# sacs-epfl/decentralizepy

Measured on AMD Instinct MI355X. Metric: GiB/s fp32 params encoded+decoded (device-resident), 1% top-k, higher is better.
Workload: dtype f32

## Files before the change

decentralizepy_amd/csrc/dpz_topk.h:

```cpp
#pragma once
#include <cstdlib>

#include "dpz_common.h"
#include "dpz_replace.h"

namespace dpz {

struct KeySrc {
  const float* x;
  const float* x0;
  float* acc;
  int mode;
  int rekey;
};

struct Raw4 {
  float4 a, b, q;
  int cnt;
};

template <bool VEC, bool ACC = true>
__device__ __forceinline__ void load_raw4(const KeySrc& s, int64_t i0, int64_t n, Raw4& r) {
  const int64_t rem = n - i0;
  r.cnt = rem >= 4 ? 4 : (rem > 0 ? (int)rem : 0);
// ... 89 lines not shown
constexpr int EX_HIST_BLOCKS = 1024;
constexpr int SMP_N = 65536;
constexpr int SMP_CHUNK = 64;
constexpr int SMP_NCHUNK = SMP_N / SMP_CHUNK;
constexpr int CB_SHIFT = 20;
constexpr int CB = 2048;
#ifndef DPZ_HB
#define DPZ_HB 1024
#endif
constexpr int HB = DPZ_HB;
constexpr int HBR = HB + 1;
static_assert(HB % 256 == 0 && HB <= 1024, "fine bins: multiple of 256, at most 1024");
#ifndef DPZ_WMAX
#define DPZ_WMAX 8192
#endif
#ifndef DPZ_WMIN_RANGE
#define DPZ_WMIN_RANGE 1024
#endif
#ifndef DPZ_FG
#define DPZ_FG 2
#endif
constexpr int W_MAX = DPZ_WMAX;
#ifndef DPZ_WSMALL
#define DPZ_WSMALL 3072
#endif
constexpr int W_SMALL = DPZ_WSMALL;
constexpr int64_t W_SMALL_N = (1 << 24) + (1 << 22);
#ifndef DPZ_WPIPE
#define DPZ_WPIPE 4096
#endif
constexpr int W_PIPE = DPZ_WPIPE;
constexpr int64_t W_PIPE_N = 1 << 24;
enum : int { GEOM_LONE = 0, GEOM_SHARED = 1, GEOM_PIPE = 2 };
constexpr int FG = DPZ_FG;
#ifndef DPZ_FOCC
#define DPZ_FOCC 8
#endif
constexpr int FOCC = DPZ_FOCC;
constexpr int W_MIN_RANGE = DPZ_WMIN_RANGE;
#ifndef DPZ_GH_COPIES
#define DPZ_GH_COPIES 8
#endif
constexpr int GH_COPIES = DPZ_GH_COPIES;
constexpr int GH_STRIDE = HB + 16;
constexpr int SEL_SEGS = 32;
constexpr int SEL_LCAP = 1024;
constexpr int NSUB = 16;
constexpr int SUBCAP = 256;
constexpr int BCAP = NSUB * SUBCAP;
constexpr int RANK_MAX = 1024;
constexpr int B_MAX = W_MAX / 4;
constexpr int STAGE = 256;
constexpr uint32_t DENSE = 0xFFFFFFFFu;

struct FastGeom {
  int64_t W;
  int64_t B;
  int64_t R;
  int64_t CAP;
};

static inline FastGeom fast_geom(int64_t n, int64_t k = 0, int geom = GEOM_LONE) {
  FastGeom g;
  int64_t W = (n + W_MIN_RANGE - 1) / W_MIN_RANGE;
  const int64_t wlone = DPZ_KNOB_INT(WLONE, 0);
  const int64_t wpipe_knob = DPZ_KNOB_INT(WPIPE, 0);
  const int64_t wpipe = (wpipe_knob > 0 && wpipe_knob <= W_MAX)
                            ? wpipe_knob
                            : (n >= W_PIPE_N ? (int64_t)W_PIPE : (int64_t)W_SMALL);
  const int64_t wmax = (geom != GEOM_LONE && n <= W_SMALL_N)
                           ? (geom == GEOM_PIPE ? wpipe : (int64_t)W_SMALL)
                           : ((wlone > 0 && wlone < W_MAX) ? wlone : W_MAX);
  if (W > wmax) W = wmax;
  if (W < 1) W = 1;
  int64_t R = (n + W - 1) / W;
  R = (R + 31) & ~int64_t(31);
  W = (n + R - 1) / R;
  int64_t cap = ((R / 4) + 63) & ~int64_t(63);
  if (k > n / 16) {
    const double frac = 1.25 * (double)k / (double)n + 0.05;
    cap = ((int64_t)(frac * (double)R) + 63) & ~int64_t(63);
    if (cap > ((R + 63) & ~int64_t(63))) cap = (R + 63) & ~int64_t(63);
  }
  if (cap < 64) cap = 64;
  if (k <= n / 16 && cap > 1024) cap = 1024;
  g.W = W; g.B = (W + 3) / 4; g.R = R; g.CAP = cap;
  return g;
}

static inline size_t align256(size_t v) { return (v + 255) & ~size_t(255); }

struct WsLayout {
  size_t ctrl, chist, ex_hist, ex_gt, ex_eq, ex_off, ex_eqb;
  size_t f_ghist, f_segcnt, f_blkabove, f_blkoff, f_cidx, f_ckey, f_cval, f_blcnt, f_blkey, f_blidx;
  size_t total;
  int64_t ex_nblk;
  FastGeom fg;
};

static inline WsLayout ws_layout(int64_t n, int64_t k = 0, int geom = GEOM_LONE) {
  WsLayout L;
  size_t o = 0;
  L.ex_nblk = (n + EX_CHUNK - 1) / EX_CHUNK;
  if (L.ex_nblk < 1) L.ex_nblk = 1;
  L.fg = fast_geom(n > 0 ? n : 1, k, geom);
  L.ctrl = o; o += align256(sizeof(TopkCtrl));
  L.chist = o; o += align256(CB * 4);
  L.ex_hist = o; o += align256(4096 * 4);
  L.ex_gt = o; o += align256(L.ex_nblk * 4);
  L.ex_eq = o; o += align256(L.ex_nblk * 4);
  L.ex_off = o; o += align256(L.ex_nblk * 4);
  L.ex_eqb = o; o += align256(L.ex_nblk * 4);
  L.f_ghist = o; o += align256(GH_COPIES * GH_STRIDE * 4);
  L.f_blcnt = o; o += align256(NSUB * 4);
  L.f_segcnt = o; o += align256(L.fg.W * 4);
  L.f_blkabove = o; o += align256(L.fg.B * 4);
  L.f_blkoff = o; o += align256(L.fg.B * 4);
  L.f_cidx = o; o += align256((size_t)L.fg.W * L.fg.CAP * 4);
  L.f_ckey = o; o += align256((size_t)L.fg.W * L.fg.CAP * 4);
  L.f_cval = o; o += align256((size_t)L.fg.W * L.fg.CAP * 4);
  L.f_blkey = o; o += align256((size_t)BCAP * 4);
  L.f_blidx = o; o += align256((size_t)BCAP * 4);
  L.total = o;
  return L;
}

static inline size_t ws_bytes_needed(int64_t n, int64_t k) {
  size_t m = 0;
  for (int geom = GEOM_LONE; geom <= GEOM_PIPE; ++geom) {
    const size_t t = ws_layout(n, k, geom).total;
    if (t > m) m = t;
  }
  return m;
}

struct EncodeArgs {
  const float* x; const float* x0; float* acc; int acc_mode; const float* vals_src;
  int64_t n, k; int32_t* idx_out; float* val_out; int32_t* counter; char* ws;
  hipStream_t st;
  const ReplaceJob* job;
  int32_t* status_out;
  bool shared;
  int val_h;
  const FoldBase* fbase;
  float* base_out;
  uint32_t* selmask;
  uint32_t* planes;
  uint32_t hint_sig;
  bool keep_x;
};
static inline uint32_t hint_signature(int64_t n, int64_t k, int geom, int acc_mode, bool x0) {
  uint64_t h = 1469598103934665603ull;
  const uint64_t v[5] = {(uint64_t)n, (uint64_t)k, (uint64_t)geom, (uint64_t)acc_mode,
                         x0 ? 1ull : 0ull};
  for (int i = 0; i < 5; ++i) h = (h ^ v[i]) * 1099511628211ull;
  return (uint32_t)(h ^ (h >> 32)) | 1u;
}
#ifndef DPZ_HINT_DELTA
#define DPZ_HINT_DELTA 0.0625f
#endif
constexpr float HINT_LO = 1.0f - DPZ_HINT_DELTA, HINT_HI = 1.0f + DPZ_HINT_DELTA;
constexpr int64_t SL_RMAX = 8192;
static inline int64_t mask_words(int64_t n) { return (n + 31) >> 5; }
int sliced_from_idx(const EncodeArgs& a, const uint32_t* guard = nullptr);
bool fused_foldbase_ok(const EncodeArgs& a, bool vec);
int launch_fold_base(const float* x, int64_t n, const FoldBase& fb, float* out, hipStream_t st);

int run_exact(const EncodeArgs& a, const WsLayout& L, int rekey, bool vec, int keep_ties = 0,
              int64_t cap = 0);
int run_sampled(const EncodeArgs& a, const WsLayout& L, bool vec, int phases = 3);
int topk_encode_status(const float* x, const float* x0, float* acc, int acc_mode,
                       const float* vals_src, int64_t n, int64_t k, int32_t* idx_out,
                       float* val_out, int32_t* counter, void* ws, size_t ws_bytes,
// ... 25 lines not shown
```

decentralizepy_amd/csrc/dpz_topk_sampled.hip:

```cpp
#include <cstdio>
#include <cstdlib>

#include "dpz_topk.h"

namespace dpz {

#ifndef DPZ_FILTER_NT
#define DPZ_FILTER_NT 1
#endif

#ifdef DPZ_STAMPS
__device__ unsigned long long g_stamps[64];
#define STAMP_MIN(i) do { if (threadIdx.x == 0) atomicMin(&g_stamps[i], __builtin_amdgcn_s_memrealtime()); } while (0)
#define STAMP_MAX(i) do { __syncthreads(); if (threadIdx.x == 0) atomicMax(&g_stamps[i], __builtin_amdgcn_s_memrealtime()); } while (0)
#define STAMP_ONE(i) do { if (threadIdx.x == 0) g_stamps[i] = __builtin_amdgcn_s_memrealtime(); } while (0)
__device__ unsigned long long g_bst[16][4096];
#define STAMP_T0(i) do { if (threadIdx.x == 0 && blockIdx.x < 4096) g_bst[i][blockIdx.x] = __builtin_amdgcn_s_memrealtime(); } while (0)
__device__ unsigned long long g_fst[6][8192];
#define STAMP_W(i) do { const int64_t _sg = (int64_t)blockIdx.x * 4 + (threadIdx.x >> 6); if ((threadIdx.x & 63) == 0 && _sg < 8192) g_fst[i][_sg] = __builtin_amdgcn_s_memrealtime(); } while (0)
#else
#define STAMP_T0(i) do {} while (0)
#define STAMP_W(i) do {} while (0)
#define STAMP_MIN(i) do {} while (0)
#define STAMP_MAX(i) do {} while (0)
// ... 72 lines not shown
#pragma unroll
  for (int e = 0; e < 8; ++e) local += hv8[e];
  uint32_t tot;
  uint32_t before = block_excl_scan(local, wsum, &tot);
#pragma unroll
  for (int e = 0; e < 8; ++e) {
    const uint32_t bin = (uint32_t)(2047 - 8 * t - e);
    const uint32_t hv = hv8[e];
    if (r_lo <= (uint32_t)SMP_N && before < r_lo && r_lo <= before + hv) win[3] = bin;
    if (r_hi >= 1 && before < r_hi && r_hi <= before + hv) win[2] = bin;
    before += hv;
  }
  __syncthreads();
  if (t == 0) {
    const uint32_t blo = win[3], bhi = win[2];
    const uint32_t lo = (blo != 0xFFFFFFFFu) ? (blo << CB_SHIFT) : 0u;
    const uint64_t h64 = (bhi != 0xFFFFFFFFu) ? ((uint64_t)(bhi + 1) << CB_SHIFT) : (1ull << 31);
    const uint32_t hi = (uint32_t)(h64 > (1ull << 31) ? (1ull << 31) : h64);
    const uint32_t width = hi - lo;
    uint32_t sft = 0;
    while ((((uint64_t)width + (1ull << sft) - 1) >> sft) > (uint64_t)HB) ++sft;
    win[0] = lo;
    win[1] = hi;
    win[2] = sft;
  }
  __syncthreads();
}

static inline void window_ranks(int64_t n, int64_t k, uint32_t* r_lo, uint32_t* r_hi) {
  const double r_est = (double)k * SMP_N / (double)n;
  const double sd = sqrt(r_est);
  const double rlo_d = ceil(r_est + 6.0 * sd + 16.0);
  const double rhi_d = floor(r_est - 6.0 * sd - 16.0);
  *r_lo = rlo_d > SMP_N ? (uint32_t)SMP_N + 1 : (uint32_t)rlo_d;
  *r_hi = rhi_d < 1.0 ? 1u : (uint32_t)rhi_d;
}

struct WaveList {
  uint32_t* gidx;
  uint32_t* gkey;
  float* gval;
  uint32_t* stg;
  uint32_t staged;
  uint32_t flushed;

  __device__ __forceinline__ void flush(int lane, bool write, uint32_t* h, uint32_t lo, uint32_t hi,
                                        uint32_t shift) {
    __builtin_amdgcn_s_waitcnt(0xC07F);
    __builtin_amdgcn_wave_barrier();
    for (uint32_t j = lane; j < staged; j += 64) {
      const uint32_t key = stg[STAGE + j];
      atomicAdd(&h[fine_bin(key, lo, hi, shift)], 1u);
      if (write) {
        gidx[flushed + j] = stg[j];
        gkey[flushed + j] = key;
        if (gval) gval[flushed + j] = __uint_as_float(stg[2 * STAGE + j]);
      }
    }
    __builtin_amdgcn_wave_barrier();
    flushed += staged;
    staged = 0;
  }
};

template <bool VEC, bool ACC, int G>
__device__ __forceinline__ void load_groups(const KeySrc& s, int64_t base, int64_t end, int lane,
                                            Raw4 (&raw)[G]) {
  if (VEC && base + G * 256 <= end) {
    const bool rekey = ACC && s.mode == DPZ_ACC_ACCUMULATE && s.rekey;
#pragma unroll
    for (int q = 0; q < G; ++q) {
      const int64_t i0 = base + q * 256 + lane * 4;
      raw[q].cnt = 4;
      if (!rekey) {
#if DPZ_FILTER_NT
        typedef float v4f __attribute__((ext_vector_type(4)));
        const v4f va = __builtin_nontemporal_load(reinterpret_cast<const v4f*>(s.x + i0));
        raw[q].a = make_float4(va.x, va.y, va.z, va.w);
        if (s.x0) {
          const v4f vb = __builtin_nontemporal_load(reinterpret_cast<const v4f*>(s.x0 + i0));
          raw[q].b = make_float4(vb.x, vb.y, vb.z, vb.w);
        }
#else
        raw[q].a = *reinterpret_cast<const float4*>(s.x + i0);
        if (s.x0) raw[q].b = *reinterpret_cast<const float4*>(s.x0 + i0);
#endif
      }
      if (ACC && s.mode != DPZ_ACC_NONE) raw[q].q = *reinterpret_cast<const float4*>(s.acc + i0);
    }
  } else {
#pragma unroll
    for (int q = 0; q < G; ++q) {
      const int64_t i0 = base + q * 256 + lane * 4;
      raw[q].cnt = 0;
      if (i0 < end) load_raw4<VEC, ACC>(s, i0, end, raw[q]);
    }
  }
}

template <bool VEC, bool ACC, int G>
__global__ void __launch_bounds__(256, ACC ? 4 : FOCC) sampled_filter_kernel(
    KeySrc s, int64_t n, uint32_t r_lo, uint32_t r_hi, int64_t W, int64_t R, int64_t CAP,
    TopkCtrl* ctrl, const uint32_t* __restrict__ chist, uint32_t* ghist, uint32_t* segcnt,
    uint32_t* cidx, uint32_t* ckey, float* cval, float* __restrict__ copy_out) {
  __shared__ uint32_t h[HBR];
  __shared__ uint32_t win[4];
  __shared__ uint32_t wsum[16];
  __shared__ uint32_t st[4][3 * STAGE];
  STAMP_W(0);
  const int wid = threadIdx.x >> 6, lane = threadIdx.x & 63;
  for (int b = threadIdx.x; b < HBR; b += 256) h[b] = 0;
  const int64_t seg = (int64_t)blockIdx.x * 4 + wid;
  const int64_t beg = seg * R;
  const int64_t end = (beg + R < n) ? beg + R : n;
  const bool store_acc = (s.mode == DPZ_ACC_ACCUMULATE) && !s.rekey;
  uint4 cv[2];
  {
    const uint4* c4 = reinterpret_cast<const uint4*>(chist) + (510 - 2 * threadIdx.x);
    cv[0] = c4[0];
    cv[1] = c4[1];
  }
  Raw4 raw[G];
  load_groups<VEC, ACC, G>(s, beg, end, lane, raw);
  block_window(cv, r_lo, r_hi, win, wsum);
  STAMP_W(1);
  STAMP_W(2);
  const uint32_t lo = win[0], hi = win[1], shift = win[2];
  if (seg == 0 && lane == 0) {
    ctrl->lo = lo;
    ctrl->hi = hi;
    ctrl->shift = shift;
  }
  WaveList L{cidx + seg * CAP, ckey + seg * CAP, cval ? cval + seg * CAP : nullptr, st[wid], 0u,
             0u};
  uint32_t run = 0;
  bool dense = false;
  for (int64_t base = beg; base < end; base += G * 256) {
    if (base != beg) load_groups<VEC, ACC, G>(s, base, end, lane, raw);
#pragma unroll
    for (int q = 0; q < G; ++q) {
      uint32_t kq[4];
      const int cq = raw[q].cnt;
      if (copy_out) {
        const int64_t i0 = base + q * 256 + lane * 4;
        if (VEC && cq == 4) {
          typedef float v4f __attribute__((ext_vector_type(4)));
          const v4f v = {raw[q].a.x, raw[q].a.y, raw[q].a.z, raw[q].a.w};
          __builtin_nontemporal_store(v, reinterpret_cast<v4f*>(copy_out + i0));
        } else {
          const float xv[4] = {raw[q].a.x, raw[q].a.y, raw[q].a.z, raw[q].a.w};
#pragma unroll
          for (int e = 0; e < 4; ++e)
            if (e < cq) copy_out[i0 + e] = xv[e];
        }
      }
      if (cq) finish_keys4<VEC, ACC>(s, base + q * 256 + lane * 4, store_acc, raw[q], kq);
      bool f[4];
      uint32_t pre = 0, tot = 0;
#pragma unroll
      for (int e = 0; e < 4; ++e) {
        f[e] = e < cq && kq[e] >= lo;
        const uint64_t m = __ballot(f[e]);
        pre += mbcnt64(m);
        tot += (uint32_t)__popcll(m);
      }
      if (tot) {
        if (!dense && run + tot <= (uint32_t)CAP && tot <= (uint32_t)STAGE) {
          const uint32_t i0 = (uint32_t)(base + q * 256 + lane * 4);
          if (L.staged + tot > STAGE) L.flush(lane, true, h, lo, hi, shift);
          uint32_t p = L.staged + pre;
          const float xv[4] = {raw[q].a.x, raw[q].a.y, raw[q].a.z, raw[q].a.w};
#pragma unroll
          for (int e = 0; e < 4; ++e) {
            if (f[e]) {
              L.stg[p] = i0 + e;
              L.stg[STAGE + p] = kq[e];
              L.stg[2 * STAGE + p] = __float_as_uint(xv[e]);
              ++p;
            }
          }
          L.staged += tot;
        } else {
          if (!dense) L.flush(lane, false, h, lo, hi, shift);
          dense = true;
#pragma unroll
          for (int e = 0; e < 4; ++e)
            if (f[e]) atomicAdd(&h[fine_bin(kq[e], lo, hi, shift)], 1u);
// ... 108 lines not shown
  }
#pragma unroll
  for (int u = 0; u < D - 1; ++u) ld(u, u);
  if (hsig) {
    const bool ok = hS == hsig && hT > 0u && hT < 0x7F800000u;
    if (!ok) {
      if (BID == 0 && threadIdx.x == 0) {
        ctrl->status = 1;
        ctrl->hinted = 1;
        ctrl->val_h = (uint32_t)val_h;
      }
      if (CP != 0) {
        const int64_t ngc = (end4 - beg + 255) >> 8;
        for (int64_t j = 0; j < ngc; ++j) {
          const int64_t i0 = beg + j * 256 + lane * 4;
          if (i0 < end4) {
            const v4f a = xa[i0 >> 2];
            const v4f b = CP == 1 ? a : v4f{fb.of(a.x), fb.of(a.y), fb.of(a.z), fb.of(a.w)};
            __builtin_nontemporal_store(b, reinterpret_cast<v4f*>(copy_out) + (i0 >> 2));
          }
        }
        if (end4 < end && end4 + lane < end) {
          const float xv = s.x[end4 + lane];
          copy_out[end4 + lane] = CP == 1 ? xv : fb.of(xv);
        }
      }
      return;
    }
    if (BID == 0) {
      if (threadIdx.x < NSUB) blcnt[threadIdx.x] = 0;
      if (threadIdx.x == 0) {
        ctrl->status = 0;
        ctrl->nbound = 0;
        ctrl->val_h = (uint32_t)val_h;
        ctrl->hinted = 1;
      }
    }
  }
  uint32_t lo, hi, shift;
  if (hsig) {
    hint_window(hT, &lo, &hi, &shift);
  } else {
    block_window(cv, r_lo, r_hi, win, wsum);
    lo = win[0];
    hi = win[1];
    shift = win[2];
  }
  STAMP_T0(6);
  if (seg == 0 && lane == 0) {
    ctrl->lo = lo;
    ctrl->hi = hi;
    ctrl->shift = shift;
  }
  WaveList L{cidx + seg * CAP, ckey + seg * CAP, cval ? cval + seg * CAP : nullptr, M.st[wid], 0u,
             0u};
  uint32_t run = 0;
  bool dense = false;
  auto proc = [&](int64_t j, int u) {
    const int64_t i0 = beg + j * 256 + lane * 4;
    const int cq = i0 < end4 ? 4 : 0;
    if (CP == 1 && cq) __builtin_nontemporal_store(A[u], reinterpret_cast<v4f*>(copy_out) + (i0 >> 2));
    if (CP == 2 && cq) {
      const v4f b = {fb.of(A[u].x), fb.of(A[u].y), fb.of(A[u].z), fb.of(A[u].w)};
      __builtin_nontemporal_store(b, reinterpret_cast<v4f*>(copy_out) + (i0 >> 2));
    }
    const float xv[4] = {A[u].x, A[u].y, A[u].z, A[u].w};
    uint32_t kq[4];
    if (SRC == 1) {
      const float bv[4] = {B[u].x, B[u].y, B[u].z, B[u].w};
#pragma unroll
      for (int e = 0; e < 4; ++e) kq[e] = key_of(xv[e] - bv[e]);
    } else if (SRC == 2) {
      const float bv[4] = {B[u].x, B[u].y, B[u].z, B[u].w};
#pragma unroll
      for (int e = 0; e < 4; ++e) kq[e] = key_of(bv[e] + xv[e]);
    } else {
#pragma unroll
      for (int e = 0; e < 4; ++e) kq[e] = key_of(xv[e]);
    }
    stage_group(L, h, kq, xv, cq, (uint32_t)i0, lane, lo, hi, shift, CAP, run, dense);
  };
  const int64_t ng = (end4 - beg + 255) >> 8;
  for (int64_t j0 = 0; j0 < ng; j0 += D) {
#pragma unroll
    for (int u = 0; u < D; ++u) {
      ld(j0 + u + D - 1, (u + D - 1) % D);
      proc(j0 + u, u);
    }
  }
  if (end4 < end) {
    const int64_t i = end4 + lane;
    const bool v = i < end;
    float xv[4] = {0.f, 0.f, 0.f, 0.f};
    uint32_t kq[4] = {0u, 0u, 0u, 0u};
    if (v) {
      xv[0] = s.x[i];
      kq[0] = key_of(SRC == 1 ? xv[0] - s.x0[i] : (SRC == 2 ? s.acc[i] + xv[0] : xv[0]));
      if (CP == 1) copy_out[i] = xv[0];
      if (CP == 2) copy_out[i] = fb.of(xv[0]);
    }
    stage_group(L, h, kq, xv, v ? 1 : 0, (uint32_t)i, lane, lo, hi, shift, CAP, run, dense);
  }
  if (!dense) L.flush(lane, true, h, lo, hi, shift);
  __syncthreads();
  uint32_t* gcopy = ghist + (BID & (GH_COPIES - 1)) * GH_STRIDE;
  for (int b = threadIdx.x; b < HBR; b += 256) {
    const uint32_t v = h[b];
    if (v) atomicAdd(&gcopy[b], v);
  }
  if (lane == 0 && seg < W) segcnt[seg] = dense ? DENSE : run;
  STAMP_T0(7);
}

template <int SRC, int CP, int D, int OCC, bool XNT>
__global__ void __launch_bounds__(256, OCC) sampled_filter_pipe_kernel(KeySrc s, int64_t n, uint32_t r_lo, uint32_t r_hi, int64_t W, int64_t R, int64_t CAP, TopkCtrl* ctrl, const uint32_t* __restrict__ chist, uint32_t* ghist, uint32_t* segcnt, uint32_t* cidx, uint32_t* ckey, float* cval, float* __restrict__ copy_out, FoldBase fb, uint32_t hsig, uint32_t* blcnt, int val_h) {
  __shared__ FilterLds lds;
  sampled_filter_pipe_kernel_body<SRC, CP, D, OCC, XNT>(lds, s, n, r_lo, r_hi, W, R, CAP, ctrl, chist, ghist, segcnt, cidx, ckey, cval, copy_out, fb, hsig, blcnt, val_h, (uint32_t)blockIdx.x);
}

__device__ __forceinline__ bool wave_bstar(const uint32_t* gh, uint32_t above, uint32_t k,
                                           uint32_t* bstar, uint32_t* need) {
  constexpr int PL = HB / 64;
  const int lane = threadIdx.x & 63;
  uint32_t hv[PL];
  const uint4* g4 = reinterpret_cast<const uint4*>(gh) + (HB / 4 - (PL / 4) * (lane + 1));
#pragma unroll
  for (int q = 0; q < PL / 4; ++q) {
    const uint4 v = g4[PL / 4 - 1 - q];
    hv[4 * q + 0] = v.w;
    hv[4 * q + 1] = v.z;
    hv[4 * q + 2] = v.y;
    hv[4 * q + 3] = v.x;
  }
  uint32_t local = 0;
#pragma unroll
  for (int e = 0; e < PL; ++e) local += hv[e];
  uint32_t tot;
  uint32_t before = wave_excl_scan(local, &tot) + above;
  uint32_t fb = 0xFFFFFFFFu, fn = 0;
#pragma unroll
  for (int e = 0; e < PL; ++e) {
    if (before < k && k <= before + hv[e]) {
      fb = (uint32_t)(HB - 1 - PL * lane - e);
      fn = k - before;
    }
    before += hv[e];
  }
  const uint64_t m = __ballot(fb != 0xFFFFFFFFu);
  const bool ok = (above < k) && (above + tot >= k) && m != 0;
  const int src = m ? (int)__ffsll((long long)m) - 1 : 0;
  *bstar = __shfl(fb, src, 64);
  *need = __shfl(fn, src, 64);
  return ok;
}

template <int NT>
struct SelectLds {
  uint32_t gh[GH_STRIDE];
  uint32_t lkey[SEL_LCAP], lidx[SEL_LCAP];
  uint32_t fbabove[NT / 64 * 2 / 4];
  uint32_t lcnt, gbase, sb_bstar, sb_need, sb_ok;
};

template <bool VEC, int NT = 1024>
__device__ __forceinline__ void sampled_select_kernel_body(SelectLds<NT>& M, KeySrc s, int64_t n, int64_t k, int64_t W, int64_t B, int64_t R, int64_t CAP, TopkCtrl* ctrl, const uint32_t* __restrict__ ghist, const uint32_t* __restrict__ segcnt, const uint32_t* __restrict__ cidx, const uint32_t* __restrict__ ckey, uint32_t* blkabove, uint32_t* blcnt, uint32_t* blkey, uint32_t* blidx, ReplaceJob pj, const uint32_t BID) {
  static_assert(NT == 1024 || NT == 256, "select block: 1024 or 256 threads");
  constexpr int SS = NT / 64 * 2;
  constexpr int NQ = HB / NT;
  {
    const int64_t own = ((W + SEL_SEGS - 1) / SEL_SEGS) * (SEL_SEGS / SS);
    if ((int64_t)BID >= own) {
      replace_block(pj, (int64_t)BID - own);
      return;
    }
  }
  STAMP_MIN(6);
  STAMP_T0(8);
  uint32_t* const gh = M.gh;
  uint32_t* const fbabove = M.fbabove;
  uint32_t* const lkey = M.lkey;
  uint32_t* const lidx = M.lidx;
  uint32_t& lcnt = M.lcnt;
  uint32_t& gbase = M.gbase;
  uint32_t& sb_bstar = M.sb_bstar;
  uint32_t& sb_need = M.sb_need;
  uint32_t& sb_ok = M.sb_ok;
  const int t = threadIdx.x, wid = t >> 6, lane = t & 63;
  const int64_t seg0 = (int64_t)BID * SS + wid * 2;
  const uint32_t cnt0 = seg0 < W ? segcnt[seg0] : 0u;
  const uint32_t cnt1 = seg0 + 1 < W ? segcnt[seg0 + 1] : 0u;
  constexpr int PFS = 4;
  uint32_t pk[2][PFS], pi[2][PFS];
#pragma unroll
  for (int u = 0; u < 2; ++u) {
    const int64_t sg = seg0 + u;
    pk[u][0] = sg < W ? ckey[sg * CAP + lane] : 0u;
    pi[u][0] = sg < W ? cidx[sg * CAP + lane] : 0u;
  }
  const uint32_t lo = ctrl->lo, hi = ctrl->hi, shift = ctrl->shift;
  const uint32_t fstatus = ctrl->status;
  static_assert(HB == 1024, "select: NQ fine bins per thread + the above-window bin");
  static_assert((GH_COPIES & (GH_COPIES - 1)) == 0 && GH_COPIES <= 64, "one copy per lane");
  uint32_t v[GH_COPIES][NQ];
#pragma unroll
  for (int c = 0; c < GH_COPIES; ++c) {
#pragma unroll
    for (int q = 0; q < NQ; ++q) v[c][q] = ghist[c * GH_STRIDE + q * NT + t];
  }
  const uint32_t va = t < GH_COPIES ? ghist[t * GH_STRIDE + HB] : 0u;
#pragma unroll
  for (int u = 0; u < 2; ++u) {
    const int64_t sg = seg0 + u;
    const uint32_t cu = u ? cnt1 : cnt0;
#pragma unroll
    for (int c = 1; c < PFS; ++c) {
      const uint32_t j = c * 64u + lane;
      pk[u][c] = 0u;
      pi[u][c] = 0u;
      if (sg < W && cu != DENSE && j < cu) {
        pk[u][c] = ckey[sg * CAP + j];
        pi[u][c] = cidx[sg * CAP + j];
      }
    }
  }
  if (fstatus) return;
  {
    uint32_t suma = va;
#pragma unroll
    for (int d = 1; d < GH_COPIES; d <<= 1) suma += __shfl_xor(suma, d, 64);
#pragma unroll
    for (int q = 0; q < NQ; ++q) {
      uint32_t sum = 0;
#pragma unroll
      for (int c = 0; c < GH_COPIES; ++c) sum += v[c][q];
      gh[q * NT + t] = sum;
    }
    if (t == 0) gh[HB] = suma;
  }
  STAMP_T0(12);
  if (t < SS / 4) fbabove[t] = 0;
  if (t == 0) lcnt = 0;
  __syncthreads();
  if (wid == 0) {
    uint32_t bstar, need;
    const bool ok = wave_bstar(gh, gh[HB], (uint32_t)k, &bstar, &need);
    if (lane == 0) {
      sb_bstar = bstar;
      sb_need = need;
      sb_ok = ok ? 1u : 0u;
    }
  }
  __syncthreads();
  if (!sb_ok) {
    if (BID == 0 && t == 0) ctrl->status = 1;
    return;
  }
  STAMP_T0(9);
  const uint32_t bstar = sb_bstar;
  if (BID == 0 && t == 0) {
    ctrl->bstar = bstar;
    ctrl->need = sb_need;
  }
  auto append = [&](bool in, uint32_t key, uint32_t idx) {
    const uint64_t m = __ballot(in);
    if (m) {
      uint32_t base = 0;
      if (lane == 0) base = atomicAdd(&lcnt, (uint32_t)__popcll(m));
      base = __shfl(base, 0, 64);
      if (in) {
        const uint32_t p = base + mbcnt64(m);
        if (p < SEL_LCAP) {
          lkey[p] = key;
          lidx[p] = idx;
        }
      }
    }
  };
#pragma unroll
  for (int u = 0; u < 2; ++u) {
    const int64_t seg = seg0 + u;
    const uint32_t cnt = u ? cnt1 : cnt0;
    uint32_t above = 0;
    if (seg < W && cnt != DENSE) {
#pragma unroll
      for (int c = 0; c < PFS; ++c) {
        const uint32_t j = c * 64u + lane;
        if (c * 64u >= cnt) break;
        const uint32_t key = pk[u][c], idx = pi[u][c];
        const uint32_t b = j < cnt ? fine_bin(key, lo, hi, shift) : 0u;
        above += (uint32_t)__popcll(__ballot(j < cnt && b > bstar));
        append(j < cnt && b == bstar, key, idx);
      }
      for (uint32_t j0 = PFS * 64u; j0 < cnt; j0 += 4 * 64u) {
        uint32_t kg[4];
#pragma unroll
        for (int g = 0; g < 4; ++g) {
          const uint32_t j = j0 + g * 64u + lane;
          kg[g] = ckey[seg * CAP + (j < cnt ? j : 0u)];
        }
#pragma unroll
        for (int g = 0; g < 4; ++g) {
          const uint32_t j = j0 + g * 64u + lane;
          const bool v = j < cnt;
          const uint32_t b = v ? fine_bin(kg[g], lo, hi, shift) : 0u;
          above += (uint32_t)__popcll(__ballot(v && b > bstar));
          const bool ap = v && b == bstar;
          const uint32_t idx = ap ? cidx[seg * CAP + j] : 0u;
          append(ap, kg[g], idx);
        }
      }
    } else if (seg < W) {
      const int64_t beg = seg * R;
      const int64_t end = (beg + R < n) ? beg + R : n;
      for (int64_t i0 = beg + lane * 4; i0 - lane * 4 < end; i0 += 256) {
        uint32_t key[4];
        const int c = i0 < end ? load_keys4<VEC>(s, i0, end, false, key) : 0;
#pragma unroll
        for (int e = 0; e < 4; ++e) {
          const bool valid = e < c && key[e] >= lo;
          const uint32_t b = valid ? fine_bin(key[e], lo, hi, shift) : 0u;
          above += (uint32_t)__popcll(__ballot(valid && b > bstar));
          append(valid && b == bstar, key[e], (uint32_t)(i0 + e));
        }
      }
    }
    if (lane == 0 && above) atomicAdd(&fbabove[(wid * 2 + u) >> 2], above);
  }
  __syncthreads();
  if (t < SS / 4) {
    const int64_t fb = (int64_t)BID * (SS / 4) + t;
    blkabove[fb] = fb < B ? fbabove[t] : 0u;
  }
  STAMP_T0(10);
  const uint32_t nl = lcnt;
  if (nl) {
    const int sub = (int)(BID & (NSUB - 1));
    if (t == 0) gbase = atomicAdd(&blcnt[sub], nl > SEL_LCAP ? (uint32_t)BCAP : nl);
    __syncthreads();
    const uint32_t gb = gbase;
    for (uint32_t j = t; j < nl && j < SEL_LCAP; j += NT) {
      const uint32_t p = gb + j;
      if (p < SUBCAP) {
        blkey[sub * SUBCAP + p] = lkey[j];
        blidx[sub * SUBCAP + p] = lidx[j];
      }
    }
  }
  STAMP_T0(11);
}

template <bool VEC>
__global__ void __launch_bounds__(1024) sampled_select_kernel(KeySrc s, int64_t n, int64_t k, int64_t W, int64_t B, int64_t R, int64_t CAP, TopkCtrl* ctrl, const uint32_t* __restrict__ ghist, const uint32_t* __restrict__ segcnt, const uint32_t* __restrict__ cidx, const uint32_t* __restrict__ ckey, uint32_t* blkabove, uint32_t* blcnt, uint32_t* blkey, uint32_t* blidx, ReplaceJob pj) {
  __shared__ __attribute__((aligned(16))) SelectLds<1024> lds;
  sampled_select_kernel_body<VEC>(lds, s, n, k, W, B, R, CAP, ctrl, ghist, segcnt, cidx, ckey, blkabove, blcnt, blkey, blidx, pj, (uint32_t)blockIdx.x);
}

__device__ __forceinline__ uint32_t bound_slot(const uint32_t* subbase, uint32_t j) {
  int sb = 0;
#pragma unroll
  for (int u = 1; u < NSUB; ++u) sb += subbase[u] <= j ? 1 : 0;
// ... 265 lines not shown
  uint64_t* const wsum64 = M.wsum64;
  ResolveLds& RL = M.RL;
  uint32_t* const bsk = M.bsk;
  uint32_t* const bsi = M.bsi;
  const int64_t CB_ = (W + CSEG - 1) / CSEG;
  const int64_t B = (W + 3) / 4;
  if (nrep_first > 0 ? (int64_t)BID < nrep_first : (int64_t)BID >= CB_) {
    replace_block(pj, nrep_first > 0 ? (int64_t)BID : (int64_t)BID - CB_);
    return;
  }
  const uint32_t blk = (uint32_t)((int64_t)BID - (nrep_first > 0 ? nrep_first : 0));
  STAMP_T0(0);
  const int t = threadIdx.x, wid = t >> 6, lane = t & 63;
  for (int64_t b = (int64_t)blk * 256 + t; b < (int64_t)GH_COPIES * GH_STRIDE; b += CB_ * 256)
    ghist[b] = 0u;
  const int64_t seg0 = (int64_t)blk * CSEG + wid * SPW;
  const uint32_t status = ctrl->status;
  const uint32_t need_l = ctrl->need, lo_l = ctrl->lo, shift_l = ctrl->shift,
                 bstar_l = ctrl->bstar;
  const uint32_t sc = t < NSUB ? blcnt[t] : 0u;
  constexpr uint32_t SPEC = 256 / NSUB;
  static_assert(NSUB * SPEC == 256 && SPEC <= SUBCAP, "one speculative entry per thread");
  const uint32_t sp_sub = (uint32_t)t / SPEC, sp_slot = (uint32_t)t % SPEC;
  const uint32_t spk = blkey[sp_sub * SUBCAP + sp_slot], spi = blidx[sp_sub * SUBCAP + sp_slot];
  static_assert(B_MAX <= 256 * 8, "above counts: 8 per thread");
  uint32_t abv_before = 0, abv_all = 0;
  {
    const uint32_t fb0 = (uint32_t)t * 8u;
    uint4 v0 = make_uint4(0, 0, 0, 0), v1 = make_uint4(0, 0, 0, 0);
    if ((int64_t)fb0 < B) {
      v0 = reinterpret_cast<const uint4*>(blkabove)[2 * t];
      v1 = reinterpret_cast<const uint4*>(blkabove)[2 * t + 1];
    }
    const uint32_t v[8] = {v0.x, v0.y, v0.z, v0.w, v1.x, v1.y, v1.z, v1.w};
    const uint32_t fbx = blk * (uint32_t)(CSEG / 4);
#pragma unroll
    for (int q = 0; q < 8; ++q) {
      abv_all += v[q];
      abv_before += fb0 + q < fbx ? v[q] : 0u;
    }
  }
  uint32_t cnt[SPW], kk[SPW][PFC], ii[SPW][PFC];
  float vv[SPW][PFC];
#pragma unroll
  for (int u = 0; u < SPW; ++u) {
    const int64_t seg = seg0 + u;
    cnt[u] = seg < W ? segcnt[seg] : 0u;
#pragma unroll
    for (int c = 0; c < PFC; ++c) {
      kk[u][c] = 0u;
      ii[u][c] = 0u;
      vv[u][c] = 0.f;
    }
    kk[u][0] = seg < W ? ckey[seg * CAP + lane] : 0u;
    ii[u][0] = seg < W ? cidx[seg * CAP + lane] : 0u;
    if (cval && seg < W) vv[u][0] = cval[seg * CAP + lane];
  }
  if (blk == 0) {
    for (int b = t; b < CB; b += 256) chist[b] = 0;
  }
  if (status) {
    if (blk == 0 && t == 0) {
      atomicOr(&ctrl->sticky, status);
      if (status_out) *status_out = (int32_t)status;
    }
    return;
  }
  uint32_t cc[SPW][PFC];
#pragma unroll
  for (int u = 0; u < SPW; ++u)
#pragma unroll
    for (int c = 0; c < PFC; ++c) cc[u][c] = 0u;
#pragma unroll
  for (int u = 0; u < SPW; ++u) {
    const int64_t seg = seg0 + u;
    if (seg < W && cnt[u] != DENSE && (uint32_t)lane < cnt[u]) {
      if (!cval) vv[u][0] = vals_src[ii[u][0]];
      if (PLAIN && counter) cc[u][0] = (uint32_t)counter[ii[u][0]];
    }
  }
  if (t < 64) {
    uint32_t tot;
    const uint32_t ex = wave_excl_scan(sc, &tot);
    const bool over = __ballot(sc > (uint32_t)SUBCAP) != 0;
    const bool spec_ok = __ballot(sc > SPEC) == 0;
    if (t < NSUB) subbase[t] = ex;
    if (t == 0) {
      subbase[NSUB] = tot;
      flag = (over || tot > (uint32_t)BCAP || need_l == 0 || need_l > tot) ? 1u : 0u;
      spec = spec_ok ? 1u : 0u;
    }
  }
  __syncthreads();
  if (flag) {
    if (blk == 0 && t == 0) {
      ctrl->status = 1;
      atomicOr(&ctrl->sticky, 1u);
      if (status_out) *status_out = 1;
    }
    return;
  }
  const uint32_t need = __builtin_amdgcn_readfirstlane(need_l);
  const uint32_t lo = __builtin_amdgcn_readfirstlane(lo_l);
  const uint32_t shift = __builtin_amdgcn_readfirstlane(shift_l);
  const uint32_t bstar = __builtin_amdgcn_readfirstlane(bstar_l);
#pragma unroll
  for (int u = 0; u < SPW; ++u) cnt[u] = __builtin_amdgcn_readfirstlane(cnt[u]);
  STAMP_T0(1);
  Bound bd{blkey, blidx, subbase, bsk, bsi, subbase[NSUB]};
  if (spec) {
    if (sp_slot < subbase[sp_sub + 1] - subbase[sp_sub]) {
      bsk[subbase[sp_sub] + sp_slot] = spk;
      bsi[subbase[sp_sub] + sp_slot] = spi;
    }
    __syncthreads();
  } else {
    bd.load();
  }
  uint32_t T, icut;
  block_resolve(bd, need, lo + (bstar << shift), shift, RL, &T, &icut);
  T = __builtin_amdgcn_readfirstlane(T);
  icut = __builtin_amdgcn_readfirstlane(icut);
  STAMP_T0(2);
  const uint32_t bstart = (uint32_t)((int64_t)blk * CSEG * R);
  uint32_t sb_before = 0, sb_all = 0;
  bd.each([&](uint32_t kv, uint32_t iv) {
    const bool sel = kv > T || (kv == T && iv <= icut);
    sb_all += sel ? 1u : 0u;
    sb_before += (sel && iv < bstart) ? 1u : 0u;
  });
  const uint64_t tot2 = block_sum64(((uint64_t)(abv_all + sb_all) << 32) |
                                        (uint64_t)(abv_before + sb_before), wsum64);
  const uint32_t boff = __builtin_amdgcn_readfirstlane((uint32_t)tot2);
  const uint32_t grand = __builtin_amdgcn_readfirstlane((uint32_t)(tot2 >> 32));
  if (blk == 0 && t == 0) {
    ctrl->T = T;
    ctrl->icut = icut;
    if (grand != (uint32_t)k) {
      ctrl->status = 2;
      atomicOr(&ctrl->sticky, 2u);
    } else if (T > 0u && T < 0x7F800000u) {
      ctrl->hint_T = T;
      ctrl->hint_sig = sig;
    } else {
      ctrl->hint_sig = 0u;
    }
    if (status_out) *status_out = grand != (uint32_t)k ? 2 : 0;
  }
  if (grand != (uint32_t)k) return;
  if constexpr (PFC > 1) {
#pragma unroll
    for (int u = 0; u < SPW; ++u) {
      const int64_t seg = seg0 + u;
      if (seg < W && cnt[u] != DENSE && cnt[u] > 64u) {
#pragma unroll
        for (int c = 1; c < PFC; ++c) {
          const uint32_t j = c * 64u + lane;
          if (j < cnt[u]) {
            kk[u][c] = ckey[seg * CAP + j];
            ii[u][c] = cidx[seg * CAP + j];
            if (cval) vv[u][c] = cval[seg * CAP + j];
          }
        }
#pragma unroll
        for (int c = 1; c < PFC; ++c) {
          const uint32_t j = c * 64u + lane;
          if (j < cnt[u] && !cval) vv[u][c] = vals_src[ii[u][c]];
          if (PLAIN && counter && j < cnt[u]) cc[u][c] = (uint32_t)counter[ii[u][c]];
        }
      }
    }
  }
  auto is_sel = [&](uint32_t key, uint32_t idx) { return key > T || (key == T && idx <= icut); };
#pragma unroll
  for (int u = 0; u < SPW; ++u) {
    const int64_t seg = seg0 + u;
    uint32_t mine = 0;
    if (seg < W && cnt[u] != DENSE) {
#pragma unroll
      for (int c = 0; c < PFC; ++c) {
        const uint32_t j = c * 64u + lane;
        mine += (uint32_t)__popcll(__ballot(j < cnt[u] && is_sel(kk[u][c], ii[u][c])));
      }
      for (uint32_t j0 = PFC * 64u; j0 < cnt[u]; j0 += 4 * 64u) {
        uint32_t kg[4];
#pragma unroll
        for (int g = 0; g < 4; ++g) {
          const uint32_t j = j0 + g * 64u + lane;
          kg[g] = ckey[seg * CAP + (j < cnt[u] ? j : 0u)];
        }
#pragma unroll
        for (int g = 0; g < 4; ++g) {
          const uint32_t j = j0 + g * 64u + lane;
          bool sel = false;
          if (j < cnt[u]) sel = kg[g] > T || (kg[g] == T && cidx[seg * CAP + j] <= icut);
          mine += (uint32_t)__popcll(__ballot(sel));
        }
      }
    } else if (seg < W) {
      mine = dense_count<VEC>(s, seg, R, n, lo, T, icut);
    }
    if (lane == 0) wcnt[wid * SPW + u] = mine;
  }
  __syncthreads();
  STAMP_T0(3);
  uint32_t run = boff;
  for (int w = 0; w < wid * SPW; ++w) run += wcnt[w];
  run = __builtin_amdgcn_readfirstlane(run);
  uint32_t* const slrow = SL ? M.slrows[wid] : nullptr;
#pragma unroll
  for (int u = 0; u < SPW; ++u) {
    const int64_t seg = seg0 + u;
    if (seg >= W) break;
    const int64_t segbeg = seg * R;
    const int segw = SL ? (int)((((segbeg + R < n) ? segbeg + R : n) - segbeg + 31) >> 5) : 0;
    if (SL) {
      for (int j = lane; j < segw; j += 64) slrow[j] = 0u;
      __builtin_amdgcn_wave_barrier();
    }
    if (cnt[u] != DENSE) {
      auto emit = [&](bool sel, uint32_t idx, float v, bool pre, uint32_t cw) {
        const uint64_t m = __ballot(sel);
        if (sel) {
          const uint32_t pos = run + mbcnt64(m);
          if (pos < (uint64_t)k) {
            idx_out[pos] = (int32_t)idx;
            store_val(val_out, val_h, pos, (cval || pre) ? v : vals_src[idx]);
            if (SL) atomicOr(&slrow[(idx >> 5) - (uint32_t)(segbeg >> 5)], 1u << (idx & 31));
            if (counter) {
              if (PLAIN) counter[idx] = (int32_t)(cw + 1u);
              else atomicAdd(&counter[idx], 1);
            }
            if (rewind) rewind[idx] = 0.0f;
          }
        }
        run += (uint32_t)__popcll(m);
      };
#pragma unroll
      for (int c = 0; c < PFC; ++c) {
        const uint32_t j = c * 64u + lane;
        if (c * 64u < cnt[u])
          emit(j < cnt[u] && is_sel(kk[u][c], ii[u][c]), ii[u][c], vv[u][c], true, cc[u][c]);
      }
      for (uint32_t j0 = PFC * 64u; j0 < cnt[u]; j0 += 4 * 64u) {
        uint32_t kg[4], ig[4];
        float vg[4];
#pragma unroll
        for (int g = 0; g < 4; ++g) {
          const uint32_t j = j0 + g * 64u + lane;
          const uint32_t jc = seg * CAP + (j < cnt[u] ? j : 0u);
          kg[g] = ckey[jc];
          ig[g] = cidx[jc];
          vg[g] = cval ? cval[jc] : 0.f;
        }
#pragma unroll
        for (int g = 0; g < 4; ++g) {
          const uint32_t j = j0 + g * 64u + lane;
          const bool sel = j < cnt[u] && is_sel(kg[g], ig[g]);
          const uint32_t cw = (PLAIN && counter && sel) ? (uint32_t)counter[ig[g]] : 0u;
          emit(sel, ig[g], vg[g], false, cw);
        }
      }
    } else {
      dense_write<VEC>(s, seg, R, n, k, lo, T, icut, run, vals_src, idx_out, val_out, counter,
                       rewind, val_h, slrow);
      run += wcnt[wid * SPW + u];
    }
    if (SL) {
      __builtin_amdgcn_fence(__ATOMIC_RELEASE, "wavefront");
      __builtin_amdgcn_wave_barrier();
      for (int j = lane; j < segw; j += 64) {
        const uint32_t m = slrow[j];
        const int64_t w = (segbeg >> 5) + j;
        selmask[w] = m;
        uint32_t carry = planes ? m : 0u;
        for (int p = 0; p < 32 && carry != 0u; p += SL_PF) {
          uint32_t o[SL_PF];
#pragma unroll
          for (int q = 0; q < SL_PF; ++q) o[q] = planes[(int64_t)(p + q) * nwords + w];
#pragma unroll
          for (int q = 0; q < SL_PF; ++q) {
            if (carry != 0u) {
              planes[(int64_t)(p + q) * nwords + w] = o[q] ^ carry;
              carry &= o[q];
            }
          }
        }
      }
      __builtin_amdgcn_wave_barrier();
    }
  }
  STAMP_T0(4);
}

template <bool VEC, bool PLAIN, int SPW, bool SL>
__global__ void __launch_bounds__(256, SPW >= 8 ? 1 : 4) sampled_compact_kernel(KeySrc s, int64_t n, int64_t k, int64_t W, int64_t R, int64_t CAP, TopkCtrl* ctrl, uint32_t* chist, const uint32_t* __restrict__ blkabove, const uint32_t* __restrict__ blcnt, const uint32_t* __restrict__ blkey, const uint32_t* __restrict__ blidx, const uint32_t* __restrict__ segcnt, const uint32_t* __restrict__ cidx, const uint32_t* __restrict__ ckey, const float* __restrict__ cval, const float* vals_src, int32_t* idx_out, float* val_out, int32_t* counter, float* rewind, int32_t* status_out, ReplaceJob pj, int64_t nrep_first, int val_h, uint32_t* selmask, uint32_t* planes, int64_t nwords, uint32_t* ghist, uint32_t sig) {
  __shared__ __attribute__((aligned(16))) CompactLds<SPW, SL> lds;
  sampled_compact_kernel_body<VEC, PLAIN, SPW, SL>(lds, s, n, k, W, R, CAP, ctrl, chist, blkabove, blcnt, blkey, blidx, segcnt, cidx, ckey, cval, vals_src, idx_out, val_out, counter, rewind, status_out, pj, nrep_first, val_h, selmask, planes, nwords, ghist, sig, (uint32_t)blockIdx.x);
}

static void cosched_shares(double f[3]) {
  f[0] = 0.45; f[1] = 0.55; f[2] = 0.0;
  if (const char* e = DPZ_KNOB_STR(COSCHED)) {
// ... 316 lines not shown
struct PipeSelectPart {
  const float* x;
  const float* x0;
  TopkCtrl* ctrl;
  const uint32_t* ghist;
  const uint32_t* segcnt;
  const uint32_t* cidx;
  const uint32_t* ckey;
  uint32_t* blkabove;
  uint32_t* blcnt;
  uint32_t* blkey;
  uint32_t* blidx;
};
struct PipeCompactPart {
  const float* x;
  const float* x0;
  TopkCtrl* ctrl;
  uint32_t* chist;
  const uint32_t* blkabove;
  const uint32_t* blcnt;
  const uint32_t* blkey;
  const uint32_t* blidx;
  const uint32_t* segcnt;
  const uint32_t* cidx;
  const uint32_t* ckey;
  const float* cval;
  uint32_t* ghist;
  int32_t* idx_out;
  float* val_out;
  int32_t* counter;
  ReplaceJob pj;
};

template <bool FILTER>
union PipeLds {
  FilterLds f;
  SelectLds<256> s;
  CompactLds<2, false> c;
};
template <>
union PipeLds<false> {
  SelectLds<256> s;
  CompactLds<2, false> c;
};

constexpr int PIPE_OCC = 5;
#ifdef DPZ_DIAG
constexpr bool PIPE_DIAG = true;
#else
constexpr bool PIPE_DIAG = false;
#endif

template <bool FILTER, int OCC>
__global__ void __launch_bounds__(256, OCC) pipe_step_kernel(
    KeySrc fs, TopkCtrl* f_ctrl, const uint32_t* __restrict__ f_chist, uint32_t* f_ghist,
    uint32_t* f_segcnt, uint32_t* f_cidx, uint32_t* f_ckey, float* f_cval, uint32_t* f_blcnt,
    float* __restrict__ f_out, uint32_t f_hsig,
    KeySrc ss, TopkCtrl* s_ctrl, const uint32_t* __restrict__ s_ghist,
    const uint32_t* __restrict__ s_segcnt, const uint32_t* __restrict__ s_cidx,
    const uint32_t* __restrict__ s_ckey, uint32_t* s_blkabove, uint32_t* s_blcnt,
    uint32_t* s_blkey, uint32_t* s_blidx,
    KeySrc cs, TopkCtrl* c_ctrl, uint32_t* c_chist, const uint32_t* __restrict__ c_blkabove,
    const uint32_t* __restrict__ c_blcnt, const uint32_t* __restrict__ c_blkey,
    const uint32_t* __restrict__ c_blidx, const uint32_t* __restrict__ c_segcnt,
    const uint32_t* __restrict__ c_cidx, const uint32_t* __restrict__ c_ckey,
    const float* __restrict__ c_cval, uint32_t* c_ghist, int32_t* c_idx_out, float* c_val_out,
    int32_t* c_counter, ReplaceJob c_pj,
    int64_t n, int64_t k, uint32_t r_lo, uint32_t r_hi, int64_t W, int64_t B, int64_t R,
    int64_t CAP, uint32_t nc, uint32_t nsel, uint32_t nf, uint32_t sig, uint32_t poison) {
  __shared__ __attribute__((aligned(16))) PipeLds<FILTER> lds;
  static_assert(sizeof(lds) % 4 == 0, "the arena is poisoned in 32-bit words");
  if (PIPE_DIAG && poison) {
    uint32_t* const w = reinterpret_cast<uint32_t*>(&lds);
    for (uint32_t j = 0; j < (uint32_t)(sizeof(lds) / 4); ++j) w[j] = 0xFFFFFFFFu;
    __syncthreads();
  }
  uint32_t bid = blockIdx.x;
  if constexpr (FILTER) {
    if (nf) {
      if (bid < nf) {
        sampled_filter_pipe_kernel_body<1, 1, 4, 4, true>(
            lds.f, fs, n, r_lo, r_hi, W, R, CAP, f_ctrl, f_chist, f_ghist, f_segcnt, f_cidx,
            f_ckey, f_cval, f_out, FoldBase{}, f_hsig, f_blcnt, 0, bid);
        return;
      }
      bid -= nf;
    }
  }
  if (bid < nc) {
    sampled_compact_kernel_body<true, false, 2, false>(
        lds.c, cs, n, k, W, R, CAP, c_ctrl, c_chist, c_blkabove, c_blcnt, c_blkey, c_blidx,
        c_segcnt, c_cidx, c_ckey, c_cval, cs.x, c_idx_out, c_val_out, c_counter, nullptr, nullptr,
        c_pj, 0, 0, nullptr, nullptr, 0, c_ghist, sig, bid);
    return;
  }
  bid -= nc;
  if (bid < nsel) {
    sampled_select_kernel_body<true, 256>(lds.s, ss, n, k, W, B, R, CAP, s_ctrl, s_ghist,
                                          s_segcnt, s_cidx, s_ckey, s_blkabove, s_blcnt, s_blkey,
                                          s_blidx, ReplaceJob{}, bid);
    return;
  }
  bid -= nsel;
  if constexpr (FILTER) {
    if (nf) return;
    sampled_filter_pipe_kernel_body<1, 1, 4, 4, true>(
        lds.f, fs, n, r_lo, r_hi, W, R, CAP, f_ctrl, f_chist, f_ghist, f_segcnt, f_cidx, f_ckey,
// ... 121 lines not shown
```

Before: 1522.

## Interleave candidate idx/key/val arrays in 32-element groups and defer index loads

Replaces the three separate per-segment candidate arrays (index, key, value) with one interleaved buffer in which each group of 32 entries stores indices, keys and values back to back. All producers and consumers in the filter, select and compact stages are updated to index through cl_off/cl_seg. This aims to put the three fields of a candidate in the same or nearby cache lines. The select stage also stops prefetching indices and loads them only for entries that fall in the boundary bin, unless the SEL_IDX_AHEAD macro is set. The pipe kernel's launch bounds become an explicit waves_per_eu(OCC,OCC) attribute, which may change register allocation.

Result: no change. 1519 (-0.2%).

```diff
diff --git a/decentralizepy_amd/csrc/dpz_topk.h b/decentralizepy_amd/csrc/dpz_topk.h
--- a/decentralizepy_amd/csrc/dpz_topk.h
+++ b/decentralizepy_amd/csrc/dpz_topk.h
@@ -165,6 +165,14 @@
 constexpr int B_MAX = W_MAX / 4;
 constexpr int STAGE = 256;
 constexpr uint32_t DENSE = 0xFFFFFFFFu;
+constexpr int CL_GROUP = 32;
+constexpr int CL_KEY = CL_GROUP, CL_VAL = 2 * CL_GROUP;
+__host__ __device__ __forceinline__ uint32_t cl_off(uint32_t j) {
+  return (j / CL_GROUP) * (3 * CL_GROUP) + (j % CL_GROUP);
+}
+__host__ __device__ __forceinline__ size_t cl_seg(int64_t seg, int64_t CAP) {
+  return (size_t)seg * 3u * (size_t)CAP;
+}
 
 struct FastGeom {
   int64_t W;
@@ -229,9 +237,10 @@
   L.f_segcnt = o; o += align256(L.fg.W * 4);
   L.f_blkabove = o; o += align256(L.fg.B * 4);
   L.f_blkoff = o; o += align256(L.fg.B * 4);
-  L.f_cidx = o; o += align256((size_t)L.fg.W * L.fg.CAP * 4);
-  L.f_ckey = o; o += align256((size_t)L.fg.W * L.fg.CAP * 4);
-  L.f_cval = o; o += align256((size_t)L.fg.W * L.fg.CAP * 4);
+  L.f_cidx = o;
+  L.f_ckey = o + CL_KEY * 4;
+  L.f_cval = o + CL_VAL * 4;
+  o += 3 * align256((size_t)L.fg.W * L.fg.CAP * 4);
   L.f_blkey = o; o += align256((size_t)BCAP * 4);
   L.f_blidx = o; o += align256((size_t)BCAP * 4);
   L.total = o;
diff --git a/decentralizepy_amd/csrc/dpz_topk_sampled.hip b/decentralizepy_amd/csrc/dpz_topk_sampled.hip
--- a/decentralizepy_amd/csrc/dpz_topk_sampled.hip
+++ b/decentralizepy_amd/csrc/dpz_topk_sampled.hip
@@ -148,9 +148,10 @@
       const uint32_t key = stg[STAGE + j];
       atomicAdd(&h[fine_bin(key, lo, hi, shift)], 1u);
       if (write) {
-        gidx[flushed + j] = stg[j];
-        gkey[flushed + j] = key;
-        if (gval) gval[flushed + j] = __uint_as_float(stg[2 * STAGE + j]);
+        const uint32_t o = cl_off(flushed + j);
+        gidx[o] = stg[j];
+        gkey[o] = key;
+        if (gval) gval[o] = __uint_as_float(stg[2 * STAGE + j]);
       }
     }
     __builtin_amdgcn_wave_barrier();
@@ -227,8 +228,8 @@
     ctrl->hi = hi;
     ctrl->shift = shift;
   }
-  WaveList L{cidx + seg * CAP, ckey + seg * CAP, cval ? cval + seg * CAP : nullptr, st[wid], 0u,
-             0u};
+  WaveList L{cidx + cl_seg(seg, CAP), ckey + cl_seg(seg, CAP),
+             cval ? cval + cl_seg(seg, CAP) : nullptr, st[wid], 0u, 0u};
   uint32_t run = 0;
   bool dense = false;
   for (int64_t base = beg; base < end; base += G * 256) {
@@ -443,8 +444,8 @@
     ctrl->hi = hi;
     ctrl->shift = shift;
   }
-  WaveList L{cidx + seg * CAP, ckey + seg * CAP, cval ? cval + seg * CAP : nullptr, M.st[wid], 0u,
-             0u};
+  WaveList L{cidx + cl_seg(seg, CAP), ckey + cl_seg(seg, CAP),
+             cval ? cval + cl_seg(seg, CAP) : nullptr, M.st[wid], 0u, 0u};
   uint32_t run = 0;
   bool dense = false;
   auto proc = [&](int64_t j, int u) {
@@ -544,6 +545,11 @@
   *need = __shfl(fn, src, 64);
   return ok;
 }
+
+#ifndef DPZ_SEL_IDX_AHEAD
+#define DPZ_SEL_IDX_AHEAD 0
+#endif
+constexpr bool SEL_IDX_AHEAD = DPZ_SEL_IDX_AHEAD != 0;
 
 template <int NT>
 struct SelectLds {
@@ -585,8 +591,8 @@
 #pragma unroll
   for (int u = 0; u < 2; ++u) {
     const int64_t sg = seg0 + u;
-    pk[u][0] = sg < W ? ckey[sg * CAP + lane] : 0u;
-    pi[u][0] = sg < W ? cidx[sg * CAP + lane] : 0u;
+    pk[u][0] = sg < W ? ckey[cl_seg(sg, CAP) + cl_off(lane)] : 0u;
+    pi[u][0] = (SEL_IDX_AHEAD && sg < W) ? cidx[cl_seg(sg, CAP) + cl_off(lane)] : 0u;
   }
   const uint32_t lo = ctrl->lo, hi = ctrl->hi, shift = ctrl->shift;
   const uint32_t fstatus = ctrl->status;
@@ -609,8 +615,8 @@
       pk[u][c] = 0u;
       pi[u][c] = 0u;
       if (sg < W && cu != DENSE && j < cu) {
-        pk[u][c] = ckey[sg * CAP + j];
-        pi[u][c] = cidx[sg * CAP + j];
+        pk[u][c] = ckey[cl_seg(sg, CAP) + cl_off(j)];
+        if (SEL_IDX_AHEAD) pi[u][c] = cidx[cl_seg(sg, CAP) + cl_off(j)];
       }
     }
   }
@@ -677,17 +683,20 @@
       for (int c = 0; c < PFS; ++c) {
         const uint32_t j = c * 64u + lane;
         if (c * 64u >= cnt) break;
-        const uint32_t key = pk[u][c], idx = pi[u][c];
+        const uint32_t key = pk[u][c];
         const uint32_t b = j < cnt ? fine_bin(key, lo, hi, shift) : 0u;
         above += (uint32_t)__popcll(__ballot(j < cnt && b > bstar));
-        append(j < cnt && b == bstar, key, idx);
+        const bool ap = j < cnt && b == bstar;
+        uint32_t idx = pi[u][c];
+        if (!SEL_IDX_AHEAD) idx = ap ? cidx[cl_seg(seg, CAP) + cl_off(j)] : 0u;
+        append(ap, key, idx);
       }
       for (uint32_t j0 = PFS * 64u; j0 < cnt; j0 += 4 * 64u) {
         uint32_t kg[4];
 #pragma unroll
         for (int g = 0; g < 4; ++g) {
           const uint32_t j = j0 + g * 64u + lane;
-          kg[g] = ckey[seg * CAP + (j < cnt ? j : 0u)];
+          kg[g] = ckey[cl_seg(seg, CAP) + cl_off(j < cnt ? j : 0u)];
         }
 #pragma unroll
         for (int g = 0; g < 4; ++g) {
@@ -696,7 +705,7 @@
           const uint32_t b = v ? fine_bin(kg[g], lo, hi, shift) : 0u;
           above += (uint32_t)__popcll(__ballot(v && b > bstar));
           const bool ap = v && b == bstar;
-          const uint32_t idx = ap ? cidx[seg * CAP + j] : 0u;
+          const uint32_t idx = ap ? cidx[cl_seg(seg, CAP) + cl_off(j)] : 0u;
           append(ap, kg[g], idx);
         }
       }
@@ -1068,9 +1077,9 @@
       ii[u][c] = 0u;
       vv[u][c] = 0.f;
     }
-    kk[u][0] = seg < W ? ckey[seg * CAP + lane] : 0u;
-    ii[u][0] = seg < W ? cidx[seg * CAP + lane] : 0u;
-    if (cval && seg < W) vv[u][0] = cval[seg * CAP + lane];
+    kk[u][0] = seg < W ? ckey[cl_seg(seg, CAP) + cl_off(lane)] : 0u;
+    ii[u][0] = seg < W ? cidx[cl_seg(seg, CAP) + cl_off(lane)] : 0u;
+    if (cval && seg < W) vv[u][0] = cval[cl_seg(seg, CAP) + cl_off(lane)];
   }
   if (blk == 0) {
     for (int b = t; b < CB; b += 256) chist[b] = 0;
@@ -1173,9 +1182,9 @@
         for (int c = 1; c < PFC; ++c) {
           const uint32_t j = c * 64u + lane;
           if (j < cnt[u]) {
-            kk[u][c] = ckey[seg * CAP + j];
-            ii[u][c] = cidx[seg * CAP + j];
-            if (cval) vv[u][c] = cval[seg * CAP + j];
+            kk[u][c] = ckey[cl_seg(seg, CAP) + cl_off(j)];
+            ii[u][c] = cidx[cl_seg(seg, CAP) + cl_off(j)];
+            if (cval) vv[u][c] = cval[cl_seg(seg, CAP) + cl_off(j)];
           }
         }
 #pragma unroll
@@ -1203,13 +1212,14 @@
 #pragma unroll
         for (int g = 0; g < 4; ++g) {
           const uint32_t j = j0 + g * 64u + lane;
-          kg[g] = ckey[seg * CAP + (j < cnt[u] ? j : 0u)];
+          kg[g] = ckey[cl_seg(seg, CAP) + cl_off(j < cnt[u] ? j : 0u)];
         }
 #pragma unroll
         for (int g = 0; g < 4; ++g) {
           const uint32_t j = j0 + g * 64u + lane;
           bool sel = false;
-          if (j < cnt[u]) sel = kg[g] > T || (kg[g] == T && cidx[seg * CAP + j] <= icut);
+          if (j < cnt[u])
+            sel = kg[g] > T || (kg[g] == T && cidx[cl_seg(seg, CAP) + cl_off(j)] <= icut);
           mine += (uint32_t)__popcll(__ballot(sel));
         }
       }
@@ -1264,7 +1274,7 @@
 #pragma unroll
         for (int g = 0; g < 4; ++g) {
           const uint32_t j = j0 + g * 64u + lane;
-          const uint32_t jc = seg * CAP + (j < cnt[u] ? j : 0u);
+          const size_t jc = cl_seg(seg, CAP) + cl_off(j < cnt[u] ? j : 0u);
           kg[g] = ckey[jc];
           ig[g] = cidx[jc];
           vg[g] = cval ? cval[jc] : 0.f;
@@ -1687,7 +1697,9 @@
 #endif
 
 template <bool FILTER, int OCC>
-__global__ void __launch_bounds__(256, OCC) pipe_step_kernel(
+__global__ void
+__attribute__((amdgpu_flat_work_group_size(1, 256), amdgpu_waves_per_eu(OCC, OCC)))
+pipe_step_kernel(
     KeySrc fs, TopkCtrl* f_ctrl, const uint32_t* __restrict__ f_chist, uint32_t* f_ghist,
     uint32_t* f_segcnt, uint32_t* f_cidx, uint32_t* f_ckey, float* f_cval, uint32_t* f_blcnt,
     float* __restrict__ f_out, uint32_t f_hsig,
```
